# zackLiuzz/MY_ORB_SLAM2

Hardware: AMD Instinct MI355X
Metric: frames/sec ORB extract+match, KITTI 1241×376 stereo, 1/2/4/8 GPU (higher is better)
Workload: dtype u8

## Files before the change

### include/orbx.h

```cpp
#ifndef ORBX_H
#define ORBX_H

#include <stddef.h>
#include <stdint.h>

#ifdef __cplusplus
extern "C" {
#endif

typedef enum {
    ORBX_OK = 0,
    ORBX_ERR_INVALID = -1,
    ORBX_ERR_DEVICE = -2,
    ORBX_ERR_CAPACITY = -3,
    ORBX_ERR_UNSUPPORTED = -4,
    ORBX_ERR_STATE = -5
} orbx_status;

typedef struct {
    float x, y;
    float size;
    float angle;
    float response;
    int32_t octave;
// ... 137 lines not shown

typedef struct {
    int32_t octree_threads;
    int32_t packed;
    int32_t ncap, kcap;
    int32_t spatial;
    int32_t fast_cells_per_wave;
    int32_t chain;
    int32_t nlevels;
    int32_t cand_cap[16];
    int32_t nfeat[16];
} orbx_regime_info;
orbx_status orbx_extractor_regime_info(const orbx_extractor* h, int batch, int in_place,
                                       orbx_regime_info* out);

const char* orbx_version(void);
const char* orbx_last_error(void);
orbx_status orbx_device_count(int* n);

#ifdef __cplusplus
}
#endif
#endif
```

### my_orb_slam2_amd/_lib.py

```python
from __future__ import annotations

import ctypes
import pathlib

import numpy as np

PKG = pathlib.Path(__file__).resolve().parent
LIB_PATH = PKG / "liborbx.so"
ORBX_LIB_ENV = "ORBX_LIB"

KEYPOINT_DTYPE = np.dtype([("x", "<f4"), ("y", "<f4"), ("size", "<f4"), ("angle", "<f4"),
                           ("response", "<f4"), ("octave", "<i4"), ("class_id", "<i4")])

KERNELS = ["k_level", "k_fast", "k_octree", "k_orient_desc", "k_stereo", "k_level0"]
MATCH_KERNELS = ["k_bow", "k_triangulate", "k_proj_search", "k_proj_resolve", "k_distinctive",
                 "k_bf"]

STATUS = {0: "ORBX_OK", -1: "ORBX_ERR_INVALID", -2: "ORBX_ERR_DEVICE", -3: "ORBX_ERR_CAPACITY",
          -4: "ORBX_ERR_UNSUPPORTED", -5: "ORBX_ERR_STATE"}


class OrbxError(RuntimeError):
    def __init__(self, fn, code):
        super().__init__(f"{fn} failed: {STATUS.get(code, code)}")
# ... 15 lines not shown
                ("level_pitch", ctypes.c_int * 16), ("level_off", ctypes.c_size_t * 16)]


class HostPyramid(ctypes.Structure):
    _fields_ = [("nlevels", ctypes.c_int), ("data", ctypes.c_void_p * 16),
                ("width", ctypes.c_int * 16), ("height", ctypes.c_int * 16),
                ("step", ctypes.c_size_t * 16)]


class RegimeInfo(ctypes.Structure):
    _fields_ = [("octree_threads", ctypes.c_int32), ("packed", ctypes.c_int32),
                ("ncap", ctypes.c_int32), ("kcap", ctypes.c_int32), ("spatial", ctypes.c_int32),
                ("fast_cells_per_wave", ctypes.c_int32), ("chain", ctypes.c_int32),
                ("nlevels", ctypes.c_int32), ("cand_cap", ctypes.c_int32 * 16),
                ("nfeat", ctypes.c_int32 * 16)]


class BfLaunchInfo(ctypes.Structure):
    _fields_ = [("chunk", ctypes.c_int32), ("nchunks", ctypes.c_int32),
                ("query_blocks", ctypes.c_int32), ("nqpad", ctypes.c_int32),
                ("merge_slice", ctypes.c_int32), ("partial_bytes", ctypes.c_int64)]


_vp, _i, _f, _sz = ctypes.c_void_p, ctypes.c_int, ctypes.c_float, ctypes.c_size_t
SIGNATURES = {
    "orbx_extractor_create": (_i, [ctypes.POINTER(ExtractorParams), ctypes.POINTER(_vp)]),
    "orbx_extractor_destroy": (_i, [_vp]),
    "orbx_extractor_tables": (_i, [_vp, _vp, _vp, _vp, _vp, _vp]),
    "orbx_extractor_prepare": (_i, [_vp, _i, _i, _i, ctypes.POINTER(_i)]),
    "orbx_extract": (_i, [_vp, _vp, _i, _i, _sz, _vp, _i, _vp, ctypes.POINTER(_i)]),
# ... 19 lines not shown
    "orbx_stereo_match_batch_device": (_i, [_vp, _vp, _f, _f, _vp, _vp, _vp, _vp]),
    "orbx_stereo_frames_device": (_i, [_vp, _vp, _vp, _i, _i, _i, _sz, _sz, _f, _f, _vp, _vp,
                                       _vp, _vp]),
    "orbx_descriptor_distance": (_i, [_vp, _vp]),
    "orbx_version": (ctypes.c_char_p, []),
    "orbx_last_error": (ctypes.c_char_p, []),
    "orbx_device_count": (_i, [ctypes.POINTER(_i)]),
    "orbx_extractor_set_overlap": (_i, [_vp, _i, _i, _i]),
    "orbx_extractor_get_overlap": (_i, [_vp, ctypes.POINTER(_i), ctypes.POINTER(_i),
                                        ctypes.POINTER(_i)]),
    "orbx_profile_enable": (_i, [_vp, _i]),
    "orbx_profile_collect": (_i, [_vp, _vp, _vp]),
    "orbx_kernel_name": (ctypes.c_char_p, [_i]),
    "orbx_extractor_launch_info": (_i, [_vp, _i, _vp, ctypes.POINTER(_i)]),
    "orbx_extractor_regime_info": (_i, [_vp, _i, _i, ctypes.POINTER(RegimeInfo)]),
    "orbx_matcher_create": (_i, [_vp, ctypes.POINTER(_vp)]),
    "orbx_matcher_destroy": (_i, [_vp]),
    "orbx_compute_three_maxima": (None, [_vp, _i, _vp, _vp, _vp]),
    "orbx_search_by_bow_kf_frame": (_i, [_vp, _vp, _vp, _vp, _vp, _vp]),
    "orbx_search_by_bow_kf_kf": (_i, [_vp, _vp, _vp, _vp, _vp, _vp, _vp]),
    "orbx_search_for_triangulation": (_i, [_vp, _vp, _vp, _vp, _vp, _vp, _f, _f, _vp, _vp, _i,
                                           _i, _vp, _i, _vp]),
    "orbx_search_by_projection": (_i, [_vp, _i, _vp, _vp, _vp, _vp, _i, _vp, _i, _i, _vp, _vp]),
    "orbx_search_by_projection_ex": (_i, [_vp, _i, _vp, _vp, _vp, _vp, _vp, _i, _vp, _i, _i, _i,
                                          _vp, _vp]),
    "orbx_search_by_sim3": (_i, [_vp, _vp, _vp, _vp, _vp, _i, _vp, _vp, _i, _vp, _vp]),
    "orbx_search_for_initialization": (_i, [_vp, _vp, _vp, _vp, _i, _vp, _vp]),
    "orbx_search_by_bow_kf_frame_batch_device": (_i, [_vp, _vp, _vp, _vp, _vp, _vp]),
    "orbx_search_for_triangulation_batch_device": (_i, [_vp, _vp, _i, _vp, _vp, _vp, _vp, _vp,
                                                        _vp, _i, _i, _vp, _vp, _vp, _vp]),
# ... 157 lines not shown
```

### my_orb_slam2_amd/csrc/orbx_capi.hip

```cpp
#include <hip/hip_runtime.h>

#include <algorithm>
#include <chrono>
#include <condition_variable>
#include <cfloat>
#include <climits>
#include <cmath>
#include <cstdio>
#include <cstdlib>
#include <cstring>
#include <functional>
#include <map>
#include <memory>
#include <mutex>
#include <shared_mutex>
#include <thread>
#include <vector>

#include "../../include/orbx.h"
#include "orbx_internal.h"
#include "orbx_kernels.h"

#ifndef ORBX_SRC_HASH
#define ORBX_SRC_HASH "0000000000000000"
// ... 440 lines not shown
    if (lds > 150 * 1024) return;
    G.chain_gx = gx;
    G.chain_gy = gy;
    G.chain_buf = (int)r16(buf);
    G.chain_rs = (int)r16(rs);
    G.chain_lds = (int)lds;
    while (h->ltab.size() % 16) h->ltab.push_back(0);
    G.chain_tab = (int)h->ltab.size();
    h->ltab.insert(h->ltab.end(), (const uint8_t*)rects.data(), (const uint8_t*)(rects.data() + rects.size()));
    while (h->ltab.size() % 16) h->ltab.push_back(0);
    G.chain_toffs = (int)h->ltab.size();
    h->ltab.insert(h->ltab.end(), (const uint8_t*)toffs.data(), (const uint8_t*)(toffs.data() + toffs.size()));
    G.chain_ok = 1;
}

orbx_status build_geometry(orbx_extractor* h, int W, int H) {
    Geometry& G = h->hg;
    memset(&G, 0, sizeof(G));
    for (int i = 0; i < 3; ++i)
        if (h->taps[i] != h->taps[6 - i]) return ORBX_ERR_UNSUPPORTED;
    h->cells.clear();
    h->rtab.clear();
    const int L = h->prm.nlevels;
    G.width = W;
    G.height = H;
    G.nlevels = L;
    G.ini_th = std::min(std::max(h->prm.ini_th_fast, 0), 255);
    G.min_th = std::min(std::max(h->prm.min_th_fast, 0), 255);
    memcpy(G.taps, h->taps, sizeof(G.taps));
    memcpy(G.umax, h->umax, sizeof(G.umax));
// ... 4 lines not shown
    for (int l = 0; l < L; ++l) {
        LevelGeom& lv = G.lv[l];
        lv.w = cvRound((float)W * h->inv_scale[l]);
        lv.h = cvRound((float)H * h->inv_scale[l]);
        if (lv.w <= 0 || lv.h <= 0) return ORBX_ERR_UNSUPPORTED;
        if (lv.w > 4096 + 32 || lv.h > 4096 + 32) return ORBX_ERR_UNSUPPORTED;
        lv.pitch = (int)align_up(lv.w + 4, 64);
        lv.off = off;
        off += (long long)align_up((size_t)lv.pitch * align_up((size_t)lv.h, 4), 256);
        lv.scale = h->scale[l];
        lv.inv_scale = h->inv_scale[l];
        lv.nfeat = h->nfeat[l];
        lv.patch_size = (int)(31 * h->scale[l]);
        const int minB = ORBX_MIN_BORDER;
        const int maxBX = lv.w - ORBX_EDGE + 3, maxBY = lv.h - ORBX_EDGE + 3;
        const float width = (float)(maxBX - minB), height = (float)(maxBY - minB);
        const int nCols = (int)(width / 30.f), nRows = (int)(height / 30.f);
        lv.ncols = nCols;
        lv.nrows = nRows;
        lv.cell_begin = (int)h->cells.size();
        lv.cand_off = cand;
        int lcap = 0;
        if (nCols > 0 && nRows > 0) {
            const int wCell = (int)std::ceil(width / nCols);
            const int hCell = (int)std::ceil(height / nRows);
            lv.wcell = wCell;
            lv.hcell = hCell;
            for (int i = 0; i < nRows; i++) {
                const float iniY = (float)(minB + i * hCell);
                float maxY = iniY + hCell + 6;
                if (iniY >= maxBY - 3) continue;
                if (maxY > maxBY) maxY = (float)maxBY;
                for (int j = 0; j < nCols; j++) {
                    const float iniX = (float)(minB + j * wCell);
                    float maxX = iniX + wCell + 6;
                    if (iniX >= maxBX - 6) continue;
                    if (maxX > maxBX) maxX = (float)maxBX;
                    CellDesc c;
                    memset(&c, 0, sizeof(c));
                    c.level = (int16_t)l;
                    c.ini_x = (int16_t)(int)iniX;
                    c.ini_y = (int16_t)(int)iniY;
                    c.cols = (int16_t)((int)maxX - (int)iniX);
                    c.rows = (int16_t)((int)maxY - (int)iniY);
                    const int dh = c.rows - 6, dw = c.cols - 6;
                    c.cap = (dh > 0 && dw > 0) ? ((dw + 1) / 2) * ((dh + 1) / 2) : 0;
                    c.slot = (int32_t)cand;
                    cand += c.cap;
                    lcap += c.cap;
                    {
                        const int lpc = std::max((c.cols + 6 + 3) / 4, fast_lpitch((3 + c.cols + 3) / 4, dw));
                        const int rows_w = std::max((int)c.rows, 4 * FAST_PF2D);
                        G.max_roi_bytes = std::max(G.max_roi_bytes, rows_w * lpc * 4);
                    }
                    if (dh > 0 && dw > 0) {
                        G.max_mbuf_bytes = std::max(G.max_mbuf_bytes, ((dh + 2) * (dw + 2) + 3) & ~3);
                        G.max_cell_px = std::max(G.max_cell_px, dh * dw);
                    }
                    if (dw > 64 || dh > 511) return ORBX_ERR_UNSUPPORTED;
                    h->cells.push_back(c);
                }
            }
        }
        lv.ncells = (int)h->cells.size() - lv.cell_begin;
        lv.cand_cap = lcap;
        G.max_ncand_level = std::max(G.max_ncand_level, lcap);
        lv.n_ini = 0;
        lv.hx = 0.f;
        if (maxBY - minB > 0) {
            const float r = std::round(static_cast<float>(maxBX - minB) / (maxBY - minB));
            if (r >= 1.f && r < 4096.f) {
                lv.n_ini = (int)r;
                lv.hx = static_cast<float>(maxBX - minB) / lv.n_ini;
            }
        }
        lv.out_cap = std::max(std::max(lv.nfeat + 3, 4 * lv.n_ini), 4);
// ... 256 lines not shown
            return ORBX_ERR_DEVICE;
        if (!HIPOK(hipStreamSynchronize(st))) return ORBX_ERR_DEVICE;
        if (!HIPOK(prepare_kernels(std::max(h->octree_lds, h->octree_lds_small), h->stereo_lds,
                                   std::max(h->level_lds, (size_t)h->hg.chain_lds), fast_lds_bytes(h->hg))))
            return ORBX_ERR_DEVICE;
        h->have_geom = true;
        h->cap_batch = 0;
    }
    if (batch > h->cap_batch) {
        if (!wait_idle(h)) return ORBX_ERR_DEVICE;
        h->pyr_images = 0;
        h->last_valid = false;
        ++h->serial;
        const Geometry& G = h->hg;
        const size_t B = (size_t)batch;
        const size_t pyr_slack = (size_t)4 * FAST_PF2D * G.lv[0].pitch + 256;
        bool ok = h->d_pyr.ensure(B * G.pyr_bytes + pyr_slack) &&
                  h->d_blur.ensure(B * G.pyr_bytes) &&
                  h->d_ccnt.ensure(B * std::max(G.n_cells, 1) * 4) &&
                  h->d_cand.ensure(B * G.cand_words * 4) &&
                  h->d_ocnt.ensure(B * G.nlevels * 4) && h->d_okp.ensure(B * G.out_words * 6) &&
                  h->d_kscr.ensure(B * h->kscratch_per_image);
        const size_t o_kps = align_up(B * 4, 256);
        const size_t o_desc = o_kps + align_up(B * G.kp_cap * sizeof(orbx_keypoint), 256);
        const size_t o_end = o_desc + B * G.kp_cap * 32;
        h->o_stereo = align_up(o_end, 256);
        ok = ok && h->d_outs.ensure(h->o_stereo + 256 + 8 * (size_t)G.kp_cap);
        if (!ok) return ORBX_ERR_DEVICE;
        uint8_t* ob = h->d_outs.as<uint8_t>();
        h->d_nkp.view(ob, B * 4);
        h->d_kps.view(ob + o_kps, B * G.kp_cap * sizeof(orbx_keypoint));
// ... 468 lines not shown
    out->octree_threads = octree_threads(batch, G.nlevels);
    out->packed = small ? 0 : 1;
    out->ncap = h->ncap;
    out->kcap = small ? h->kcap_small : h->kcap;
    out->spatial = orient_spatial(batch) ? 1 : 0;
    out->fast_cells_per_wave = fast_cells_per_wave(G.n_cells, batch, h->ncu);
    out->chain = chain_of(h, in_place ? 1 : 0, side_mode_of(h, batch), batch);
    out->nlevels = G.nlevels;
    for (int l = 0; l < G.nlevels; ++l) {
        out->cand_cap[l] = G.lv[l].cand_cap;
        out->nfeat[l] = G.lv[l].nfeat;
    }
    return ORBX_OK;
}

orbx_status orbx_device_count(int* n) {
    if (!n) return ORBX_ERR_INVALID;
    int c = 0;
    if (!HIPOK(hipGetDeviceCount(&c))) { *n = 0; return ORBX_ERR_DEVICE; }
    *n = c;
    return ORBX_OK;
}

int orbx_descriptor_distance(const uint8_t* a, const uint8_t* b) {
    int d = 0;
    for (int i = 0; i < 32; ++i) d += __builtin_popcount((unsigned)(a[i] ^ b[i]));
    return d;
}

static hipError_t create_side_stream(hipStream_t* s) {
// ... 684 lines not shown
```

### my_orb_slam2_amd/csrc/orbx_extract.hip

```cpp
#include <hip/hip_runtime.h>

#include <mutex>
#include <type_traits>
#include <stdint.h>

#include "orbx_device.h"
#include "orbx_internal.h"
#include "orbx_math.h"
#include "orbx_kernels.h"

namespace orbx {

__constant__ __attribute__((aligned(4))) int8_t c_pattern[1024] = {
#include "orbx_pattern.inc"
};

typedef _Float16 f16x2 __attribute__((ext_vector_type(2)));
__device__ __forceinline__ f16x2 arc_y(const uint8_t* p) {
    const _Float16 f = __builtin_bit_cast(_Float16, (unsigned short)*p);
    return f16x2{-f, f};
}
__device__ __forceinline__ int fast_arc_score_pk(const uint8_t* roi, int cols, int r, int c) {
    const uint8_t* p = roi + r * cols + c;
    const int v = p[0];
// ... 11 lines not shown
    f16x2 m3[16], m9[16];
#pragma unroll
    for (int i = 0; i < 16; ++i) m3[i] = PMN3(y[i], y[(i + 1) & 15], y[(i + 2) & 15]);
#pragma unroll
    for (int i = 0; i < 16; ++i) m9[i] = PMN3(m3[i], m3[(i + 3) & 15], m3[(i + 6) & 15]);
    f16x2 b = PMX3(m9[0], m9[1], m9[2]);
#pragma unroll
    for (int i = 3; i < 15; i += 2) b = PMX3(b, m9[i], m9[i + 1]);
    b = __builtin_elementwise_maximum(b, m9[15]);
#undef PMN3
#undef PMX3
    const uint32_t bits = __builtin_bit_cast(uint32_t, b);
    return max(v - (int)(bits & 0x3FFu), (int)((bits >> 16) & 0x3FFu) - v);
}

__device__ __forceinline__ void fast_nms_kp2(const uint8_t* mb, int mw, int rr, int cc, int t_hi,
                                             int t_lo, bool& k_hi, bool& k_lo, int& score) {
    const uint8_t* p = mb + (rr + 1) * mw + (cc + 1);
    const int m = p[0], s = m - 1;
    score = s;
    const int q0 = p[-mw - 1], q1 = p[-mw], q2 = p[-mw + 1], q3 = p[-1], q4 = p[1];
    const int q5 = p[mw - 1], q6 = p[mw], q7 = p[mw + 1];
    int supp = 0;
#define ORBX_NB(q) supp = max(supp, (q) >= m ? (q) : 0);
    ORBX_NB(q0) ORBX_NB(q1) ORBX_NB(q2) ORBX_NB(q3) ORBX_NB(q4) ORBX_NB(q5) ORBX_NB(q6) ORBX_NB(q7)
#undef ORBX_NB
    const bool base = s > 0;
    k_hi = base && m > t_hi && supp <= t_hi;
    k_lo = base && m > t_lo && supp <= t_lo;
}

#define FAST_PF 6
#define FAST_WPE 6
#define OCT_NT 128
#define OCT_NT_SMALL 256
#define OD_SPATIAL_MIN_BATCH 16
#define OD_SP_XS 5
#define OD_SP_YS 5
#define OD_WPE 5
__device__ __forceinline__ void lds_order() { __asm__ volatile("" ::: "memory"); }

typedef unsigned short u16x2 __attribute__((ext_vector_type(2)));

__device__ __forceinline__ u16x2 pair_u16(const uint32_t* A, int s_abs) {
// ... 1 lines not shown
    const uint32_t sel = (uint32_t)s | 0x0C00u | (uint32_t)(s + 1) << 16 | 0x0C000000u;
    return __builtin_bit_cast(u16x2, __builtin_amdgcn_perm(A[k + 1], A[k], sel));
}

__device__ __forceinline__ uint32_t pair_u16_stride2(const uint32_t* A, int s_abs) {
    const int k = s_abs >> 2, s = s_abs & 3;
    const uint32_t sel = (uint32_t)s | 0x0C00u | (uint32_t)(s + 2) << 16 | 0x0C000000u;
    return __builtin_amdgcn_perm(A[k + 1], A[k], sel);
}

#define CMP_B0 14
#define CMP_B1 15
#define CMP_B2 30
#define CMP_B3 31

template <int XO>
__device__ __forceinline__ uint32_t compass4_fr(const uint8_t* roi0, int rp, int R, int gx, uint32_t K) {
    const uint8_t* row = roi0 + __umul24((uint32_t)R, (uint32_t)rp);
    const uint32_t* rc = (const uint32_t*)row + gx;
    const uint32_t* rd = (const uint32_t*)(row + 3 * rp) + gx;
    const uint32_t* ru = (const uint32_t*)(row - 3 * rp) + gx;
    constexpr int KC = (XO + 9) >> 2;
    constexpr int K0 = (XO + 3) >> 2, K1 = (XO + 6) >> 2;
    uint32_t C[5], D[5], U[5];
#pragma unroll
    for (int k = 0; k < 5; ++k) {
        C[k] = k <= KC ? rc[k] : 0u;
        D[k] = (k >= K0 && k <= K1) ? rd[k] : 0u;
        U[k] = (k >= K0 && k <= K1) ? ru[k] : 0u;
    }
    uint32_t F[2];
#pragma unroll
    for (int h = 0; h < 2; ++h) {
        const int o = XO + 3 + h;
        const uint32_t V = pair_u16_stride2(C, o);
        const uint32_t N12 = pair_u16_stride2(C, o - 3), N4 = pair_u16_stride2(C, o + 3);
        const uint32_t N0 = pair_u16_stride2(D, o), N8 = pair_u16_stride2(U, o);
        const uint32_t A = K - V, B = K + V;
        const uint32_t bright = ((N0 + A) | (N8 + A)) & ((N4 + A) | (N12 + A));
        const uint32_t dark = ((B - N0) | (B - N8)) & ((B - N4) | (B - N12));
        F[h] = (bright | dark) & 0x40004000u;
    }
    return F[0] | (F[1] << 1);
}

__device__ __forceinline__ uint32_t compass_pair_mm(uint32_t V, uint32_t N0, uint32_t N4,
                                                    uint32_t N8, uint32_t N12, uint32_t K) {
    const u16x2 a0 = __builtin_bit_cast(u16x2, N0), a4 = __builtin_bit_cast(u16x2, N4);
    const u16x2 a8 = __builtin_bit_cast(u16x2, N8), a12 = __builtin_bit_cast(u16x2, N12);
    const uint32_t mb = __builtin_bit_cast(uint32_t, __builtin_elementwise_min(
        __builtin_elementwise_max(a0, a8), __builtin_elementwise_max(a4, a12)));
    const uint32_t md = __builtin_bit_cast(uint32_t, __builtin_elementwise_max(
        __builtin_elementwise_min(a0, a8), __builtin_elementwise_min(a4, a12)));
    return ((mb + (K - V)) | ((K + V) - md)) & 0x40004000u;
}

template <int XO>
__device__ __forceinline__ uint32_t compass16_fr(const uint8_t* roi0, int rp, int R, int g, uint32_t K) {
    const uint8_t* row = roi0 + __umul24((uint32_t)R, (uint32_t)rp);
    const uint4* rc = (const uint4*)row + g;
    const uint4* rd = (const uint4*)(row + 3 * rp) + g;
    const uint4* ru = (const uint4*)(row - 3 * rp) + g;
    const uint4 c0 = rc[0], c1 = rc[1], d0 = rd[0], u0 = ru[0];
    const uint2 d1 = *(const uint2*)(rd + 1), u1 = *(const uint2*)(ru + 1);
    const uint32_t C[8] = {c0.x, c0.y, c0.z, c0.w, c1.x, c1.y, c1.z, c1.w};
    const uint32_t D[6] = {d0.x, d0.y, d0.z, d0.w, d1.x, d1.y};
    const uint32_t U[6] = {u0.x, u0.y, u0.z, u0.w, u1.x, u1.y};
    uint32_t mask = 0;
#pragma unroll
// ... 33 lines not shown
    const int wid = threadIdx.x >> 6, lane = threadIdx.x & 63;
    int bx, b;
    xcd_block(bx, b);
    const int c_first = __builtin_amdgcn_readfirstlane(c_begin + (bx * 4 + wid) * nc);
    if (c_first >= c_end) return;
    const int ncw = min(nc, c_end - c_first);
    const int roi_cap = (g->max_roi_bytes + 15) & ~15, mb_cap = (g->max_mbuf_bytes + 15) & ~15;
    const int cl_cap = (g->max_cell_px * 2 + 15) & ~15;
    uint8_t* roi0 = smem + wid * (roi_cap + mb_cap + 64 * 2 + cl_cap);
    uint8_t* mb = roi0 + roi_cap;
    int16_t* list = (int16_t*)(mb + mb_cap);
    int16_t* corners = list;
    const uint8_t* pyr_b = pyr + (size_t)b * g->pyr_bytes;

    uint32_t pf[FAST_PF2D];
    const int lr2 = lane >> 4, lc2 = lane & 15;
    auto prefetch = [&](const CellDesc& c) -> bool {
        const int ndw = ((c.ini_x & 3) + c.cols + 3) >> 2;
        if (ndw > 16 || c.rows > 4 * FAST_PF2D || c.rows <= 6 || c.cols <= 6) return false;
        const LevelGeom& L = g->lv[c.level];
        const uint8_t* src = pyr_b + L.off + (size_t)c.ini_y * L.pitch + (c.ini_x & ~3);
        const uint32_t lane_off = __umul24((uint32_t)lr2, (uint32_t)L.pitch) + 4u * (uint32_t)min(lc2, ndw - 1);
        const __amdgpu_buffer_rsrc_t rs = __builtin_amdgcn_make_buffer_rsrc((void*)src, 0, 0x7FFFFFFF, 0x00020000);
#pragma unroll
        for (int j = 0; j < FAST_PF2D; ++j)
            pf[j] = __builtin_amdgcn_raw_buffer_load_b32(rs, lane_off, (uint32_t)(4 * j) * (uint32_t)L.pitch, 0);
        return true;
    };
    CellDesc cn = cells[c_first];
    bool have = prefetch(cn);
    const uint32_t wslot = (uint32_t)cn.slot;
    uint32_t wpos = 0;
    for (int k = 0; k < ncw; ++k) {
        const int ci = c_first + k;
        const CellDesc c = cn;
        const bool pre = have;
        const int rows = c.rows, cols = c.cols, dh = rows - 6, dw = cols - 6;
        int* cnt_out = ccnt + (size_t)b * g->n_cells + ci;
        const int xo = c.ini_x & 3;
        const int ndw = (xo + cols + 3) >> 2;
        const int lp = fast_lpitch(ndw, dw);
        const int rp = lp * 4;
        if (dh > 0 && dw > 0) {
            if (pre) {
                if (lc2 < ndw) {
                    uint32_t* l = (uint32_t*)roi0 + lr2 * lp + lc2;
#pragma unroll
                    for (int j = 0; j < FAST_PF2D; ++j)
                        l[4 * j * lp] = pf[j];
                }
            } else {
                const LevelGeom& L = g->lv[c.level];
                stage_dwords<64>(pyr_b + L.off + (size_t)c.ini_y * L.pitch + (c.ini_x & ~3),
                                 L.pitch, rows, ndw, (uint32_t*)roi0, lp, lane);
            }
        }
        if (k + 1 < ncw) {
            cn = cells[ci + 1];
            have = prefetch(cn);
        }
        if (dh <= 0 || dw <= 0) {
            if (lane == 0) *cnt_out = 0;
            continue;
        }
        const uint8_t* roi = roi0 + xo;
        const int mw = dw + 2;
        for (int i = lane; i < ((dh + 2) * mw + 15) >> 4; i += 64) ((uint4*)mb)[i] = make_uint4(0u, 0u, 0u, 0u);
        lds_order();
        const int gsh = ((dw + 3) >> 2) <= 8 ? 3 : 4;
        [[maybe_unused]] const int rpp = 64 >> gsh;
        const int sub = lane >> gsh, gx = lane & ((1 << gsh) - 1);
        const uint32_t colmask4 = (1u << min(max(dw - 4 * gx, 0), 4)) - 1u;
        const uint32_t colmask = ((colmask4 & 3u) << CMP_B0) | ((colmask4 & 12u) << (CMP_B2 - 2));
        [[maybe_unused]] constexpr int PB[4] = {CMP_B0, CMP_B1, CMP_B2, CMP_B3};
        const int lsh = dw > 32 ? 2 : 1;
        const int rpp16 = 64 >> lsh;
        const int sub16 = lane >> lsh, g16 = lane & ((1 << lsh) - 1);
        const int rem16 = dw - 16 * g16;
        const uint32_t colmask16 = rem16 >= 16 ? 0xFFFFu : (rem16 > 0 ? (1u << rem16) - 1u : 0u);
        const int rows_blk = rpp16;
        (void)colmask; (void)sub; (void)gx;
        uint32_t* slot = cand + (size_t)b * g->cand_words + wslot + wpos;
        const int t_ini = g->ini_th, t_min = g->min_th;
        int base = 0;
        for (int pass = 0; pass < 2; ++pass) {
        const int tq = pass == 0 ? t_ini : t_min;
        const uint32_t KT = (uint32_t)(0x4000 - tq - 1) * 0x10001u;
        int ncorner = 0;
        for (int rb = 0; rb < dh; rb += rows_blk) {
            int nlist = 0;
            {
                const int rr = rb + sub16;
                const int R = min(rr, dh - 1) + 3;
                uint32_t f;
                switch (xo) {
                    case 0: f = compass16_fr<0>(roi0, rp, R, g16, KT); break;
                    case 1: f = compass16_fr<1>(roi0, rp, R, g16, KT); break;
                    case 2: f = compass16_fr<2>(roi0, rp, R, g16, KT); break;
                    default: f = compass16_fr<3>(roi0, rp, R, g16, KT); break;
                }
                f &= rr < dh ? colmask16 : 0u;
                const int cnt = __builtin_popcount(f);
                const int incl = wave_incl_scan_dpp(cnt);
                int pos = incl - cnt;
                const int e0 = (rr << 6) | (16 * g16);
                int16_t* pl = list + ncorner;
                while (f) {
                    pl[pos++] = (int16_t)(e0 + __builtin_ctz(f));
                    f &= f - 1u;
                }
                nlist = __builtin_amdgcn_readlane(incl, 63);
            }
            lds_order();
            const int lb = ncorner;
            for (int j0 = 0; j0 < nlist; j0 += 64) {
                const int j = j0 + lane;
                int pe = 0, m = 0;
                if (j < nlist) {
                    pe = list[lb + j];
                    const int rr = pe >> 6, cc = pe & 63;
                    m = fast_arc_score_pk(roi, rp, rr + 3, cc + 3);
                    mb[(rr + 1) * mw + cc + 1] = (uint8_t)max(m, 0);
                }
                const bool corner = j < nlist && m > tq;
                const uint64_t cm = __ballot(corner);
                if (corner) corners[ncorner + lanes_below(cm)] = (int16_t)pe;
                ncorner += __popcll(cm);
            }
            lds_order();
        }
        const int th_hi = tq, th_lo = tq;
        if (ncorner <= 64) {
            int sc = 0, pe = 0;
            bool k_hi = false, k_lo = false;
            if (lane < ncorner) {
                pe = corners[lane];
                fast_nms_kp2(mb, mw, pe >> 6, pe & 63, th_hi, th_lo, k_hi, k_lo, sc);
            }
            const uint64_t mh = __ballot(k_hi);
            const bool kk = mh ? k_hi : k_lo;
            const uint64_t m = mh ? mh : __ballot(k_lo);
            if (kk) {
                const int idx = lanes_below(m);
                const int x = c.ini_x + (pe & 63) + 3 - ORBX_MIN_BORDER;
                const int y = c.ini_y + (pe >> 6) + 3 - ORBX_MIN_BORDER;
                if (idx < c.cap) slot[idx] = pack_cand(x, y, sc);
            }
            base = __popcll(m);
        } else {
            bool found = false;
            for (int j0 = 0; j0 < ncorner && !found; j0 += 64) {
                const int j = j0 + lane;
                int sc = 0;
                bool k_hi = false, k_lo = false;
                if (j < ncorner) {
                    const int pe = corners[j];
                    fast_nms_kp2(mb, mw, pe >> 6, pe & 63, th_hi, th_lo, k_hi, k_lo, sc);
                }
                found = __ballot(k_hi) != 0;
            }
            for (int j0 = 0; j0 < ncorner; j0 += 64) {
                const int j = j0 + lane;
                int sc = 0, pe = 0;
                bool k_hi = false, k_lo = false;
                if (j < ncorner) {
                    pe = corners[j];
                    fast_nms_kp2(mb, mw, pe >> 6, pe & 63, th_hi, th_lo, k_hi, k_lo, sc);
                }
                const bool kk = found ? k_hi : k_lo;
                const uint64_t m = __ballot(kk);
                if (kk) {
                    const int idx = base + lanes_below(m);
                    const int x = c.ini_x + (pe & 63) + 3 - ORBX_MIN_BORDER;
                    const int y = c.ini_y + (pe >> 6) + 3 - ORBX_MIN_BORDER;
                    if (idx < c.cap) slot[idx] = pack_cand(x, y, sc);
                }
                base += __popcll(m);
            }
        }
        if (base > 0) break;
        lds_order();
        }
        const int nout = min(base, c.cap);
        if (lane == 0) *cnt_out = nout | (int)(((uint32_t)c.slot - (wslot + wpos)) << 16);
        wpos += (uint32_t)nout;
        lds_order();
    }
}

size_t fast_lds_bytes(const Geometry& G) {
    const int roi_cap = (G.max_roi_bytes + 15) & ~15, mb_cap = (G.max_mbuf_bytes + 15) & ~15;
    const int cl_cap = (G.max_cell_px * 2 + 15) & ~15;
    return (size_t)4 * (roi_cap + mb_cap + 64 * 2 + cl_cap);
// ... 953 lines not shown
```

### my_orb_slam2_amd/csrc/orbx_internal.h

```cpp
#pragma once
#include <hip/hip_runtime.h>
#include <stdint.h>
#include <stddef.h>

#define ORBX_MAX_LEVELS 16
#define ORBX_EDGE 19
#define ORBX_MIN_BORDER 16
#define ORBX_MAX_DEVICES 64

namespace orbx {

struct LevelGeom {
    int w, h, pitch;
    long long off;
    float scale, inv_scale;
    int nfeat;
    int ncols, nrows, wcell, hcell;
    int cell_begin, ncells;
    long long cand_off;
    int cand_cap;
    int n_ini;
    float hx;
    int out_off, out_cap;
    int kp_level_cap;
// ... 96 lines not shown
    int chain_toffs;
    int chain_buf;
    int chain_rs;
    int chain_lds;
    LevelGeom lv[ORBX_MAX_LEVELS];
};

#define FAST_NC 4
#define FAST_PF2D 10
__host__ __device__ inline int fast_lpitch(int ndw, int dw) {
    const int lpr = dw > 32 ? 4 : 2;
    const int need = ndw > 4 * lpr + 4 ? ndw : 4 * lpr + 4;
    return (need + 3) & ~3;
}

__host__ __device__ inline uint32_t pack_cand(int x, int y, int score) {
    return (uint32_t)x | ((uint32_t)y << 12) | ((uint32_t)score << 24);
}
__host__ __device__ inline int cand_x(uint32_t c) { return (int)(c & 0xFFF); }
__host__ __device__ inline int cand_y(uint32_t c) { return (int)((c >> 12) & 0xFFF); }
__host__ __device__ inline int cand_s(uint32_t c) { return (int)(c >> 24); }

}
```

### my_orb_slam2_amd/extractor.py

```python
from __future__ import annotations

import ctypes

import numpy as np

from ._lib import (BatchView, ExtractorParams, HostPyramid, KERNELS, KEYPOINT_DTYPE, RegimeInfo,
                   check, load, ptr)


class _DeviceArray:

    def __init__(self, ptr_value: int, shape, strides, typestr: str = "|u1"):
        self.__cuda_array_interface__ = {"shape": tuple(shape), "typestr": typestr,
                                         "data": (int(ptr_value), False),
                                         "strides": tuple(strides), "version": 2}


class ORBextractor:

    def __init__(self, nfeatures: int = 1000, scaleFactor: float = 1.2, nlevels: int = 8,
                 iniThFAST: int = 20, minThFAST: int = 7, *, cv_simd: int = 1,
                 max_batch: int = 1, device: int = 0):
        self._L = load()
        self.params = ExtractorParams(nfeatures, scaleFactor, nlevels, iniThFAST, minThFAST,
# ... 181 lines not shown
        split = ctypes.c_int(0)
        check("orbx_extractor_launch_info", self._L.orbx_extractor_launch_info(
            self._h, batch, ptr(rows), ctypes.byref(split)))
        return rows, split.value

    def regime_info(self, batch: int, in_place: bool = False) -> dict:
        r = RegimeInfo()
        check("orbx_extractor_regime_info", self._L.orbx_extractor_regime_info(
            self._h, batch, int(in_place), ctypes.byref(r)))
        out = {k: int(getattr(r, k)) for k in ("octree_threads", "packed", "ncap", "kcap",
                                               "spatial", "fast_cells_per_wave", "chain")}
        out["cand_cap"] = [int(v) for v in r.cand_cap[:r.nlevels]]
        out["nfeat"] = [int(v) for v in r.nfeat[:r.nlevels]]
        return out

    def batch_view(self) -> BatchView:
        v = BatchView()
        check("orbx_batch_view_get", self._L.orbx_batch_view_get(self._h, ctypes.byref(v)))
        return v

    def batch_tensors(self):
        import torch
        v = self.batch_view()
        dev = torch.device("cuda", self.params.device)
        B, KC = v.batch, v.kp_cap
        kps = torch.as_tensor(_DeviceArray(v.kps, (B, KC, 28), (KC * 28, 28, 1)), device=dev)
        desc = torch.as_tensor(_DeviceArray(v.desc, (B, KC, 32), (KC * 32, 32, 1)), device=dev)
        nkp = torch.as_tensor(_DeviceArray(v.nkp, (B,), (4,), "<i4"), device=dev)
        return kps, desc, nkp

# ... 133 lines not shown
```

Before: 137,700.

## Add 5x12 FAST prefetch grid, remainder-row blocks, and single-threshold NMS pass

Cells whose ROI fits in 12 dwords now use a 5x12 lane grid covering 50 rows of register prefetch, so fewer cells fall back to the staged LDS copy. Leftover rows after the full 16-lane blocks are handled by a narrower 4-pixel compass block instead of a full block, which cuts wasted detection work. The dual-threshold NMS with an early-exit search is replaced by one loop at a single threshold. The change also adds a host-side FAST plan info API and increases pyramid slack to cover the taller prefetch window, at the cost of more branching and grid selection logic in the kernel.

```diff
diff --git a/include/orbx.h b/include/orbx.h
--- a/include/orbx.h
+++ b/include/orbx.h
@@ -175,6 +175,21 @@
 orbx_status orbx_extractor_regime_info(const orbx_extractor* h, int batch, int in_place,
                                        orbx_regime_info* out);
 
+#define ORBX_FAST_INFO_TOTAL 16
+typedef struct {
+    int32_t nlevels;
+    int32_t cells[17];
+    int32_t grid_5x12[17];
+    int32_t grid_4x16[17];
+    int32_t staged[17];
+    int32_t empty[17];
+    int32_t full_blocks[17];
+    int32_t rem_blocks[17];
+} orbx_fast_info;
+orbx_status orbx_extractor_fast_info(const orbx_extractor* h, orbx_fast_info* out);
+orbx_status orbx_fast_info_for(const orbx_extractor_params* p, int width, int height,
+                               orbx_fast_info* out);
+
 const char* orbx_version(void);
 const char* orbx_last_error(void);
 orbx_status orbx_device_count(int* n);
diff --git a/my_orb_slam2_amd/_lib.py b/my_orb_slam2_amd/_lib.py
--- a/my_orb_slam2_amd/_lib.py
+++ b/my_orb_slam2_amd/_lib.py
@@ -53,6 +53,19 @@
                 ("fast_cells_per_wave", ctypes.c_int32), ("chain", ctypes.c_int32),
                 ("nlevels", ctypes.c_int32), ("cand_cap", ctypes.c_int32 * 16),
                 ("nfeat", ctypes.c_int32 * 16)]
+
+
+FAST_INFO_FIELDS = ("cells", "grid_5x12", "grid_4x16", "staged", "empty", "full_blocks",
+                    "rem_blocks")
+
+
+class FastInfo(ctypes.Structure):
+    _fields_ = [("nlevels", ctypes.c_int32)] + [(k, ctypes.c_int32 * 17) for k in FAST_INFO_FIELDS]
+
+    def as_dict(self) -> dict:
+        out = {k: [int(v) for v in getattr(self, k)[:self.nlevels]] for k in FAST_INFO_FIELDS}
+        out["total"] = {k: int(getattr(self, k)[16]) for k in FAST_INFO_FIELDS}
+        return out
 
 
 class BfLaunchInfo(ctypes.Structure):
@@ -102,6 +115,8 @@
     "orbx_kernel_name": (ctypes.c_char_p, [_i]),
     "orbx_extractor_launch_info": (_i, [_vp, _i, _vp, ctypes.POINTER(_i)]),
     "orbx_extractor_regime_info": (_i, [_vp, _i, _i, ctypes.POINTER(RegimeInfo)]),
+    "orbx_extractor_fast_info": (_i, [_vp, ctypes.POINTER(FastInfo)]),
+    "orbx_fast_info_for": (_i, [ctypes.POINTER(ExtractorParams), _i, _i, ctypes.POINTER(FastInfo)]),
     "orbx_matcher_create": (_i, [_vp, ctypes.POINTER(_vp)]),
     "orbx_matcher_destroy": (_i, [_vp]),
     "orbx_compute_three_maxima": (None, [_vp, _i, _vp, _vp, _vp]),
diff --git a/my_orb_slam2_amd/csrc/orbx_capi.hip b/my_orb_slam2_amd/csrc/orbx_capi.hip
--- a/my_orb_slam2_amd/csrc/orbx_capi.hip
+++ b/my_orb_slam2_amd/csrc/orbx_capi.hip
@@ -478,6 +478,66 @@
     G.chain_ok = 1;
 }
 
+static bool fast_level_cells(int l, int w, int h, long long& cand, std::vector<CellDesc>& cells,
+                             int& ncols, int& nrows, int& wcell, int& hcell) {
+    const int minB = ORBX_MIN_BORDER;
+    const int maxBX = w - ORBX_EDGE + 3, maxBY = h - ORBX_EDGE + 3;
+    const float width = (float)(maxBX - minB), height = (float)(maxBY - minB);
+    const int nCols = (int)(width / 30.f), nRows = (int)(height / 30.f);
+    ncols = nCols;
+    nrows = nRows;
+    wcell = hcell = 0;
+    if (nCols <= 0 || nRows <= 0) return true;
+    const int wCell = (int)std::ceil(width / nCols);
+    const int hCell = (int)std::ceil(height / nRows);
+    wcell = wCell;
+    hcell = hCell;
+    for (int i = 0; i < nRows; i++) {
+        const float iniY = (float)(minB + i * hCell);
+        float maxY = iniY + hCell + 6;
+        if (iniY >= maxBY - 3) continue;
+        if (maxY > maxBY) maxY = (float)maxBY;
+        for (int j = 0; j < nCols; j++) {
+            const float iniX = (float)(minB + j * wCell);
+            float maxX = iniX + wCell + 6;
+            if (iniX >= maxBX - 6) continue;
+            if (maxX > maxBX) maxX = (float)maxBX;
+            CellDesc c;
+            memset(&c, 0, sizeof(c));
+            c.level = (int16_t)l;
+            c.ini_x = (int16_t)(int)iniX;
+            c.ini_y = (int16_t)(int)iniY;
+            c.cols = (int16_t)((int)maxX - (int)iniX);
+            c.rows = (int16_t)((int)maxY - (int)iniY);
+            const int dh = c.rows - 6, dw = c.cols - 6;
+            c.cap = (dh > 0 && dw > 0) ? ((dw + 1) / 2) * ((dh + 1) / 2) : 0;
+            c.slot = (int32_t)cand;
+            cand += c.cap;
+            if (dw > 64 || dh > 511) return false;
+            cells.push_back(c);
+        }
+    }
+    return true;
+}
+
+static void fast_info_of(const std::vector<CellDesc>& cells, int nlevels, orbx_fast_info* out) {
+    memset(out, 0, sizeof(*out));
+    out->nlevels = nlevels;
+    for (const CellDesc& c : cells) {
+        const FastCellPlan p = fast_cell_plan(c);
+        const bool area = c.rows > 6 && c.cols > 6;
+        int32_t* const grid = !area ? out->empty
+                              : p.grid == FAST_GRID_5x12 ? out->grid_5x12
+                              : p.grid == FAST_GRID_4x16 ? out->grid_4x16 : out->staged;
+        int32_t* const fields[] = {out->cells, grid, out->full_blocks, out->rem_blocks};
+        const int add[] = {1, 1, p.full, p.rem};
+        for (int k = 0; k < 4; ++k) {
+            fields[k][c.level] += add[k];
+            fields[k][ORBX_FAST_INFO_TOTAL] += add[k];
+        }
+    }
+}
+
 orbx_status build_geometry(orbx_extractor* h, int W, int H) {
     Geometry& G = h->hg;
     memset(&G, 0, sizeof(G));
@@ -512,52 +572,21 @@
         lv.patch_size = (int)(31 * h->scale[l]);
         const int minB = ORBX_MIN_BORDER;
         const int maxBX = lv.w - ORBX_EDGE + 3, maxBY = lv.h - ORBX_EDGE + 3;
-        const float width = (float)(maxBX - minB), height = (float)(maxBY - minB);
-        const int nCols = (int)(width / 30.f), nRows = (int)(height / 30.f);
-        lv.ncols = nCols;
-        lv.nrows = nRows;
         lv.cell_begin = (int)h->cells.size();
         lv.cand_off = cand;
+        if (!fast_level_cells(l, lv.w, lv.h, cand, h->cells, lv.ncols, lv.nrows, lv.wcell, lv.hcell))
+            return ORBX_ERR_UNSUPPORTED;
         int lcap = 0;
-        if (nCols > 0 && nRows > 0) {
-            const int wCell = (int)std::ceil(width / nCols);
-            const int hCell = (int)std::ceil(height / nRows);
-            lv.wcell = wCell;
-            lv.hcell = hCell;
-            for (int i = 0; i < nRows; i++) {
-                const float iniY = (float)(minB + i * hCell);
-                float maxY = iniY + hCell + 6;
-                if (iniY >= maxBY - 3) continue;
-                if (maxY > maxBY) maxY = (float)maxBY;
-                for (int j = 0; j < nCols; j++) {
-                    const float iniX = (float)(minB + j * wCell);
-                    float maxX = iniX + wCell + 6;
-                    if (iniX >= maxBX - 6) continue;
-                    if (maxX > maxBX) maxX = (float)maxBX;
-                    CellDesc c;
-                    memset(&c, 0, sizeof(c));
-                    c.level = (int16_t)l;
-                    c.ini_x = (int16_t)(int)iniX;
-                    c.ini_y = (int16_t)(int)iniY;
-                    c.cols = (int16_t)((int)maxX - (int)iniX);
-                    c.rows = (int16_t)((int)maxY - (int)iniY);
-                    const int dh = c.rows - 6, dw = c.cols - 6;
-                    c.cap = (dh > 0 && dw > 0) ? ((dw + 1) / 2) * ((dh + 1) / 2) : 0;
-                    c.slot = (int32_t)cand;
-                    cand += c.cap;
-                    lcap += c.cap;
-                    {
-                        const int lpc = std::max((c.cols + 6 + 3) / 4, fast_lpitch((3 + c.cols + 3) / 4, dw));
-                        const int rows_w = std::max((int)c.rows, 4 * FAST_PF2D);
-                        G.max_roi_bytes = std::max(G.max_roi_bytes, rows_w * lpc * 4);
-                    }
-                    if (dh > 0 && dw > 0) {
-                        G.max_mbuf_bytes = std::max(G.max_mbuf_bytes, ((dh + 2) * (dw + 2) + 3) & ~3);
-                        G.max_cell_px = std::max(G.max_cell_px, dh * dw);
-                    }
-                    if (dw > 64 || dh > 511) return ORBX_ERR_UNSUPPORTED;
-                    h->cells.push_back(c);
-                }
+        for (size_t k = (size_t)lv.cell_begin; k < h->cells.size(); ++k) {
+            const CellDesc& c = h->cells[k];
+            const int dh = c.rows - 6, dw = c.cols - 6;
+            lcap += c.cap;
+            const int lpc = std::max((c.cols + 6 + 3) / 4, fast_lpitch((3 + c.cols + 3) / 4, dw));
+            const int rows_w = std::max((int)c.rows, fast_roi_rows(fast_cell_plan(c).grid, c.rows));
+            G.max_roi_bytes = std::max(G.max_roi_bytes, rows_w * lpc * 4);
+            if (dh > 0 && dw > 0) {
+                G.max_mbuf_bytes = std::max(G.max_mbuf_bytes, ((dh + 2) * (dw + 2) + 3) & ~3);
+                G.max_cell_px = std::max(G.max_cell_px, dh * dw);
             }
         }
         lv.ncells = (int)h->cells.size() - lv.cell_begin;
@@ -844,7 +873,7 @@
         ++h->serial;
         const Geometry& G = h->hg;
         const size_t B = (size_t)batch;
-        const size_t pyr_slack = (size_t)4 * FAST_PF2D * G.lv[0].pitch + 256;
+        const size_t pyr_slack = (size_t)FAST_PF_ROWS * G.lv[0].pitch + 256;
         bool ok = h->d_pyr.ensure(B * G.pyr_bytes + pyr_slack) &&
                   h->d_blur.ensure(B * G.pyr_bytes) &&
                   h->d_ccnt.ensure(B * std::max(G.n_cells, 1) * 4) &&
@@ -1343,6 +1372,35 @@
     return ORBX_OK;
 }
 
+orbx_status orbx_extractor_fast_info(const orbx_extractor* h, orbx_fast_info* out) {
+    if (!h || !out) return ORBX_ERR_INVALID;
+    std::lock_guard<std::mutex> lk(h->mu);
+    if (!h->have_geom) return ORBX_ERR_STATE;
+    fast_info_of(h->cells, h->hg.nlevels, out);
+    return ORBX_OK;
+}
+
+orbx_status orbx_fast_info_for(const orbx_extractor_params* p, int width, int height,
+                               orbx_fast_info* out) {
+    if (!p || !out || width < 1 || height < 1 || p->nlevels < 1 || p->nlevels > ORBX_MAX_LEVELS ||
+        !(p->scale_factor > 0.f))
+        return ORBX_ERR_INVALID;
+    std::unique_ptr<orbx_extractor> th(new orbx_extractor());
+    orbx_extractor& t = *th;
+    t.prm = *p;
+    compute_tables(&t);
+    std::vector<CellDesc> cells;
+    long long cand = 0;
+    for (int l = 0; l < p->nlevels; ++l) {
+        const int w = cvRound((float)width * t.inv_scale[l]), hh = cvRound((float)height * t.inv_scale[l]);
+        int ncols, nrows, wcell, hcell;
+        if (w <= 0 || hh <= 0 || !fast_level_cells(l, w, hh, cand, cells, ncols, nrows, wcell, hcell))
+            return ORBX_ERR_UNSUPPORTED;
+    }
+    fast_info_of(cells, p->nlevels, out);
+    return ORBX_OK;
+}
+
 orbx_status orbx_device_count(int* n) {
     if (!n) return ORBX_ERR_INVALID;
     int c = 0;
diff --git a/my_orb_slam2_amd/csrc/orbx_extract.hip b/my_orb_slam2_amd/csrc/orbx_extract.hip
--- a/my_orb_slam2_amd/csrc/orbx_extract.hip
+++ b/my_orb_slam2_amd/csrc/orbx_extract.hip
@@ -49,8 +49,8 @@
     return max(v - (int)(bits & 0x3FFu), (int)((bits >> 16) & 0x3FFu) - v);
 }
 
-__device__ __forceinline__ void fast_nms_kp2(const uint8_t* mb, int mw, int rr, int cc, int t_hi,
-                                             int t_lo, bool& k_hi, bool& k_lo, int& score) {
+__device__ __forceinline__ bool fast_nms_kp(const uint8_t* mb, int mw, int rr, int cc, int t,
+                                            int& score) {
     const uint8_t* p = mb + (rr + 1) * mw + (cc + 1);
     const int m = p[0], s = m - 1;
     score = s;
@@ -60,9 +60,7 @@
 #define ORBX_NB(q) supp = max(supp, (q) >= m ? (q) : 0);
     ORBX_NB(q0) ORBX_NB(q1) ORBX_NB(q2) ORBX_NB(q3) ORBX_NB(q4) ORBX_NB(q5) ORBX_NB(q6) ORBX_NB(q7)
 #undef ORBX_NB
-    const bool base = s > 0;
-    k_hi = base && m > t_hi && supp <= t_hi;
-    k_lo = base && m > t_lo && supp <= t_lo;
+    return s > 0 && m > t && supp <= t;
 }
 
 #define FAST_PF 6
@@ -94,6 +92,17 @@
 #define CMP_B2 30
 #define CMP_B3 31
 
+__device__ __forceinline__ uint32_t compass_pair_mm(uint32_t V, uint32_t N0, uint32_t N4,
+                                                    uint32_t N8, uint32_t N12, uint32_t K) {
+    const u16x2 a0 = __builtin_bit_cast(u16x2, N0), a4 = __builtin_bit_cast(u16x2, N4);
+    const u16x2 a8 = __builtin_bit_cast(u16x2, N8), a12 = __builtin_bit_cast(u16x2, N12);
+    const uint32_t mb = __builtin_bit_cast(uint32_t, __builtin_elementwise_min(
+        __builtin_elementwise_max(a0, a8), __builtin_elementwise_max(a4, a12)));
+    const uint32_t md = __builtin_bit_cast(uint32_t, __builtin_elementwise_max(
+        __builtin_elementwise_min(a0, a8), __builtin_elementwise_min(a4, a12)));
+    return ((mb + (K - V)) | ((K + V) - md)) & 0x40004000u;
+}
+
 template <int XO>
 __device__ __forceinline__ uint32_t compass4_fr(const uint8_t* roi0, int rp, int R, int gx, uint32_t K) {
     const uint8_t* row = roi0 + __umul24((uint32_t)R, (uint32_t)rp);
@@ -116,23 +125,9 @@
         const uint32_t V = pair_u16_stride2(C, o);
         const uint32_t N12 = pair_u16_stride2(C, o - 3), N4 = pair_u16_stride2(C, o + 3);
         const uint32_t N0 = pair_u16_stride2(D, o), N8 = pair_u16_stride2(U, o);
-        const uint32_t A = K - V, B = K + V;
-        const uint32_t bright = ((N0 + A) | (N8 + A)) & ((N4 + A) | (N12 + A));
-        const uint32_t dark = ((B - N0) | (B - N8)) & ((B - N4) | (B - N12));
-        F[h] = (bright | dark) & 0x40004000u;
+        F[h] = compass_pair_mm(V, N0, N4, N8, N12, K);
     }
     return F[0] | (F[1] << 1);
-}
-
-__device__ __forceinline__ uint32_t compass_pair_mm(uint32_t V, uint32_t N0, uint32_t N4,
-                                                    uint32_t N8, uint32_t N12, uint32_t K) {
-    const u16x2 a0 = __builtin_bit_cast(u16x2, N0), a4 = __builtin_bit_cast(u16x2, N4);
-    const u16x2 a8 = __builtin_bit_cast(u16x2, N8), a12 = __builtin_bit_cast(u16x2, N12);
-    const uint32_t mb = __builtin_bit_cast(uint32_t, __builtin_elementwise_min(
-        __builtin_elementwise_max(a0, a8), __builtin_elementwise_max(a4, a12)));
-    const uint32_t md = __builtin_bit_cast(uint32_t, __builtin_elementwise_max(
-        __builtin_elementwise_min(a0, a8), __builtin_elementwise_min(a4, a12)));
-    return ((mb + (K - V)) | ((K + V) - md)) & 0x40004000u;
 }
 
 template <int XO>
@@ -196,27 +191,33 @@
     const uint8_t* pyr_b = pyr + (size_t)b * g->pyr_bytes;
 
     uint32_t pf[FAST_PF2D];
-    const int lr2 = lane >> 4, lc2 = lane & 15;
-    auto prefetch = [&](const CellDesc& c) -> bool {
+    int lr = 0, lc = 0;
+    auto prefetch = [&](const CellDesc& c) -> int {
         const int ndw = ((c.ini_x & 3) + c.cols + 3) >> 2;
-        if (ndw > 16 || c.rows > 4 * FAST_PF2D || c.rows <= 6 || c.cols <= 6) return false;
+        const int grid = fast_roi_grid(ndw, c.rows, c.cols);
+        if (grid == FAST_STAGED) return grid;
+        const bool g12 = grid == FAST_GRID_5x12;
+        const int lq12 = (lane * 43) >> 9;
+        lr = g12 ? (lane < 60 ? lq12 : 4) : lane >> 4;
+        lc = g12 ? (lane < 60 ? lane - 12 * lq12 : 15) : lane & 15;
         const LevelGeom& L = g->lv[c.level];
         const uint8_t* src = pyr_b + L.off + (size_t)c.ini_y * L.pitch + (c.ini_x & ~3);
-        const uint32_t lane_off = __umul24((uint32_t)lr2, (uint32_t)L.pitch) + 4u * (uint32_t)min(lc2, ndw - 1);
+        const uint32_t lane_off = __umul24((uint32_t)lr, (uint32_t)L.pitch) + 4u * (uint32_t)min(lc, ndw - 1);
+        const uint32_t rstep = (g12 ? 5u : 4u) * (uint32_t)L.pitch;
         const __amdgpu_buffer_rsrc_t rs = __builtin_amdgcn_make_buffer_rsrc((void*)src, 0, 0x7FFFFFFF, 0x00020000);
 #pragma unroll
         for (int j = 0; j < FAST_PF2D; ++j)
-            pf[j] = __builtin_amdgcn_raw_buffer_load_b32(rs, lane_off, (uint32_t)(4 * j) * (uint32_t)L.pitch, 0);
-        return true;
+            pf[j] = __builtin_amdgcn_raw_buffer_load_b32(rs, lane_off, (uint32_t)j * rstep, 0);
+        return grid;
     };
     CellDesc cn = cells[c_first];
-    bool have = prefetch(cn);
+    int have = prefetch(cn);
     const uint32_t wslot = (uint32_t)cn.slot;
     uint32_t wpos = 0;
     for (int k = 0; k < ncw; ++k) {
         const int ci = c_first + k;
         const CellDesc c = cn;
-        const bool pre = have;
+        const int pre = have;
         const int rows = c.rows, cols = c.cols, dh = rows - 6, dw = cols - 6;
         int* cnt_out = ccnt + (size_t)b * g->n_cells + ci;
         const int xo = c.ini_x & 3;
@@ -224,12 +225,13 @@
         const int lp = fast_lpitch(ndw, dw);
         const int rp = lp * 4;
         if (dh > 0 && dw > 0) {
-            if (pre) {
-                if (lc2 < ndw) {
-                    uint32_t* l = (uint32_t*)roi0 + lr2 * lp + lc2;
+            if (pre != FAST_STAGED) {
+                if (lc < ndw) {
+                    uint32_t* l = (uint32_t*)roi0 + lr * lp + lc;
+                    const int lstep = (pre == FAST_GRID_5x12 ? 5 : 4) * lp;
 #pragma unroll
                     for (int j = 0; j < FAST_PF2D; ++j)
-                        l[4 * j * lp] = pf[j];
+                        l[j * lstep] = pf[j];
                 }
             } else {
                 const LevelGeom& L = g->lv[c.level];
@@ -249,19 +251,13 @@
         const int mw = dw + 2;
         for (int i = lane; i < ((dh + 2) * mw + 15) >> 4; i += 64) ((uint4*)mb)[i] = make_uint4(0u, 0u, 0u, 0u);
         lds_order();
-        const int gsh = ((dw + 3) >> 2) <= 8 ? 3 : 4;
-        [[maybe_unused]] const int rpp = 64 >> gsh;
-        const int sub = lane >> gsh, gx = lane & ((1 << gsh) - 1);
-        const uint32_t colmask4 = (1u << min(max(dw - 4 * gx, 0), 4)) - 1u;
-        const uint32_t colmask = ((colmask4 & 3u) << CMP_B0) | ((colmask4 & 12u) << (CMP_B2 - 2));
-        [[maybe_unused]] constexpr int PB[4] = {CMP_B0, CMP_B1, CMP_B2, CMP_B3};
         const int lsh = dw > 32 ? 2 : 1;
-        const int rpp16 = 64 >> lsh;
         const int sub16 = lane >> lsh, g16 = lane & ((1 << lsh) - 1);
         const int rem16 = dw - 16 * g16;
         const uint32_t colmask16 = rem16 >= 16 ? 0xFFFFu : (rem16 > 0 ? (1u << rem16) - 1u : 0u);
-        const int rows_blk = rpp16;
-        (void)colmask; (void)sub; (void)gx;
+        const int rows_blk = 64 >> lsh;
+        int nfull, nrem;
+        fast_blocks(dh, dw, nfull, nrem);
         uint32_t* slot = cand + (size_t)b * g->cand_words + wslot + wpos;
         const int t_ini = g->ini_th, t_min = g->min_th;
         int base = 0;
@@ -269,12 +265,12 @@
         const int tq = pass == 0 ? t_ini : t_min;
         const uint32_t KT = (uint32_t)(0x4000 - tq - 1) * 0x10001u;
         int ncorner = 0;
-        for (int rb = 0; rb < dh; rb += rows_blk) {
-            int nlist = 0;
-            {
-                const int rr = rb + sub16;
+        for (int ib = 0; ib < nfull + nrem; ++ib) {
+            uint32_t f;
+            int e0;
+            if (ib < nfull) {
+                const int rr = ib * rows_blk + sub16;
                 const int R = min(rr, dh - 1) + 3;
-                uint32_t f;
                 switch (xo) {
                     case 0: f = compass16_fr<0>(roi0, rp, R, g16, KT); break;
                     case 1: f = compass16_fr<1>(roi0, rp, R, g16, KT); break;
@@ -282,17 +278,31 @@
                     default: f = compass16_fr<3>(roi0, rp, R, g16, KT); break;
                 }
                 f &= rr < dh ? colmask16 : 0u;
-                const int cnt = __builtin_popcount(f);
-                const int incl = wave_incl_scan_dpp(cnt);
-                int pos = incl - cnt;
-                const int e0 = (rr << 6) | (16 * g16);
-                int16_t* pl = list + ncorner;
-                while (f) {
-                    pl[pos++] = (int16_t)(e0 + __builtin_ctz(f));
-                    f &= f - 1u;
-                }
-                nlist = __builtin_amdgcn_readlane(incl, 63);
-            }
+                e0 = (rr << 6) | (16 * g16);
+            } else {
+                const int gsh = lsh + 2;
+                const int rr = nfull * rows_blk + (lane >> gsh), gx = lane & ((1 << gsh) - 1);
+                const int R = min(rr, dh - 1) + 3;
+                switch (xo) {
+                    case 0: f = compass4_fr<0>(roi0, rp, R, gx, KT); break;
+                    case 1: f = compass4_fr<1>(roi0, rp, R, gx, KT); break;
+                    case 2: f = compass4_fr<2>(roi0, rp, R, gx, KT); break;
+                    default: f = compass4_fr<3>(roi0, rp, R, gx, KT); break;
+                }
+                f = ((f >> CMP_B0) & 3u) | ((f >> (CMP_B2 - 2)) & 12u);
+                const uint32_t colmask4 = (1u << min(max(dw - 4 * gx, 0), 4)) - 1u;
+                f &= rr < dh ? colmask4 : 0u;
+                e0 = (rr << 6) | (4 * gx);
+            }
+            const int cnt = __builtin_popcount(f);
+            const int incl = wave_incl_scan_dpp(cnt);
+            int pos = incl - cnt;
+            int16_t* pl = list + ncorner;
+            while (f) {
+                pl[pos++] = (int16_t)(e0 + __builtin_ctz(f));
+                f &= f - 1u;
+            }
+            const int nlist = __builtin_amdgcn_readlane(incl, 63);
             lds_order();
             const int lb = ncorner;
             for (int j0 = 0; j0 < nlist; j0 += 64) {
@@ -311,54 +321,22 @@
             }
             lds_order();
         }
-        const int th_hi = tq, th_lo = tq;
-        if (ncorner <= 64) {
+        for (int j0 = 0; j0 < ncorner; j0 += 64) {
+            const int j = j0 + lane;
             int sc = 0, pe = 0;
-            bool k_hi = false, k_lo = false;
-            if (lane < ncorner) {
-                pe = corners[lane];
-                fast_nms_kp2(mb, mw, pe >> 6, pe & 63, th_hi, th_lo, k_hi, k_lo, sc);
-            }
-            const uint64_t mh = __ballot(k_hi);
-            const bool kk = mh ? k_hi : k_lo;
-            const uint64_t m = mh ? mh : __ballot(k_lo);
+            bool kk = false;
+            if (j < ncorner) {
+                pe = corners[j];
+                kk = fast_nms_kp(mb, mw, pe >> 6, pe & 63, tq, sc);
+            }
+            const uint64_t m = __ballot(kk);
             if (kk) {
-                const int idx = lanes_below(m);
+                const int idx = base + lanes_below(m);
                 const int x = c.ini_x + (pe & 63) + 3 - ORBX_MIN_BORDER;
                 const int y = c.ini_y + (pe >> 6) + 3 - ORBX_MIN_BORDER;
                 if (idx < c.cap) slot[idx] = pack_cand(x, y, sc);
             }
-            base = __popcll(m);
-        } else {
-            bool found = false;
-            for (int j0 = 0; j0 < ncorner && !found; j0 += 64) {
-                const int j = j0 + lane;
-                int sc = 0;
-                bool k_hi = false, k_lo = false;
-                if (j < ncorner) {
-                    const int pe = corners[j];
-                    fast_nms_kp2(mb, mw, pe >> 6, pe & 63, th_hi, th_lo, k_hi, k_lo, sc);
-                }
-                found = __ballot(k_hi) != 0;
-            }
-            for (int j0 = 0; j0 < ncorner; j0 += 64) {
-                const int j = j0 + lane;
-                int sc = 0, pe = 0;
-                bool k_hi = false, k_lo = false;
-                if (j < ncorner) {
-                    pe = corners[j];
-                    fast_nms_kp2(mb, mw, pe >> 6, pe & 63, th_hi, th_lo, k_hi, k_lo, sc);
-                }
-                const bool kk = found ? k_hi : k_lo;
-                const uint64_t m = __ballot(kk);
-                if (kk) {
-                    const int idx = base + lanes_below(m);
-                    const int x = c.ini_x + (pe & 63) + 3 - ORBX_MIN_BORDER;
-                    const int y = c.ini_y + (pe >> 6) + 3 - ORBX_MIN_BORDER;
-                    if (idx < c.cap) slot[idx] = pack_cand(x, y, sc);
-                }
-                base += __popcll(m);
-            }
+            base += __popcll(m);
         }
         if (base > 0) break;
         lds_order();
diff --git a/my_orb_slam2_amd/csrc/orbx_internal.h b/my_orb_slam2_amd/csrc/orbx_internal.h
--- a/my_orb_slam2_amd/csrc/orbx_internal.h
+++ b/my_orb_slam2_amd/csrc/orbx_internal.h
@@ -134,6 +134,38 @@
     return (need + 3) & ~3;
 }
 
+#define FAST_STAGED 0
+#define FAST_GRID_4x16 1
+#define FAST_GRID_5x12 2
+#define FAST_PF_ROWS (5 * FAST_PF2D)
+__host__ __device__ inline int fast_roi_grid(int ndw, int rows, int cols) {
+    if (rows <= 6 || cols <= 6) return FAST_STAGED;
+    if (ndw <= 12) return rows <= 5 * FAST_PF2D ? FAST_GRID_5x12 : FAST_STAGED;
+    return ndw <= 16 && rows <= 4 * FAST_PF2D ? FAST_GRID_4x16 : FAST_STAGED;
+}
+__host__ __device__ inline int fast_roi_rows(int grid, int rows) {
+    return grid == FAST_GRID_5x12 ? 5 * FAST_PF2D : (grid == FAST_GRID_4x16 ? 4 * FAST_PF2D : rows);
+}
+
+__host__ __device__ inline void fast_blocks(int dh, int dw, int& full, int& rem) {
+    const int sh16 = dw > 32 ? 4 : 5, rows4 = dw > 32 ? 4 : 8;
+    const int left = dh & ((1 << sh16) - 1);
+    rem = (left > 0 && left <= rows4) ? 1 : 0;
+    full = (dh >> sh16) + (left > rows4 ? 1 : 0);
+}
+
+struct FastCellPlan {
+    int grid;
+    int full, rem;
+};
+__host__ __device__ inline FastCellPlan fast_cell_plan(const CellDesc& c) {
+    FastCellPlan p;
+    p.grid = fast_roi_grid(((c.ini_x & 3) + c.cols + 3) >> 2, c.rows, c.cols);
+    p.full = p.rem = 0;
+    if (c.rows > 6 && c.cols > 6) fast_blocks(c.rows - 6, c.cols - 6, p.full, p.rem);
+    return p;
+}
+
 __host__ __device__ inline uint32_t pack_cand(int x, int y, int score) {
     return (uint32_t)x | ((uint32_t)y << 12) | ((uint32_t)score << 24);
 }
diff --git a/my_orb_slam2_amd/extractor.py b/my_orb_slam2_amd/extractor.py
--- a/my_orb_slam2_amd/extractor.py
+++ b/my_orb_slam2_amd/extractor.py
@@ -4,8 +4,17 @@
 
 import numpy as np
 
-from ._lib import (BatchView, ExtractorParams, HostPyramid, KERNELS, KEYPOINT_DTYPE, RegimeInfo,
-                   check, load, ptr)
+from ._lib import (BatchView, ExtractorParams, FastInfo, HostPyramid, KERNELS, KEYPOINT_DTYPE,
+                   RegimeInfo, check, load, ptr)
+
+
+def fast_info_for(width: int, height: int, nfeatures: int = 1000, scaleFactor: float = 1.2,
+                  nlevels: int = 8, iniThFAST: int = 20, minThFAST: int = 7) -> dict:
+    p = ExtractorParams(nfeatures, scaleFactor, nlevels, iniThFAST, minThFAST, 1, 1, 0)
+    r = FastInfo()
+    check("orbx_fast_info_for", load().orbx_fast_info_for(ctypes.byref(p), width, height,
+                                                          ctypes.byref(r)))
+    return r.as_dict()
 
 
 class _DeviceArray:
@@ -219,6 +228,11 @@
         out["nfeat"] = [int(v) for v in r.nfeat[:r.nlevels]]
         return out
 
+    def fast_info(self) -> dict:
+        r = FastInfo()
+        check("orbx_extractor_fast_info", self._L.orbx_extractor_fast_info(self._h, ctypes.byref(r)))
+        return r.as_dict()
+
     def batch_view(self) -> BatchView:
         v = BatchView()
         check("orbx_batch_view_get", self._L.orbx_batch_view_get(self._h, ctypes.byref(v)))
```

Result: no change. 138,200, median of 4 (+0.4%).
